# dotnetpower/infomesh

Hardware: AMD Instinct MI355X
Metric: queries/sec (hybrid BM25+dense search, 1.25M docs) (higher is better)
Workload: dtype bf16; 1 GPU; model=bge-small-en(random-init) encoder + BM25 CSR + cosine top-k, global_batch=128, seq_len=32, parallelism=shard1, mode=hybrid, docs_per_gpu=1250000, total_docs=1250000

## Files before the change

### infomesh_amd/index/gpu_index.py

```python
from __future__ import annotations

import math
import re
from dataclasses import dataclass

import numpy as np
import torch

from ..hashing import hash64
from .doc_attrs import DEAD_BIT, DocFilter, pack_pred, passes, words_i32

BM25_K1 = 1.2
BM25_B = 0.75
BM25_VOCAB = 1 << 17

MAX_SEGMENTS = 16

_WORD_RE = re.compile(r"\w+")


def bm25_term_ids(text: str, vocab: int = BM25_VOCAB) -> np.ndarray:
    from ..utils.plugins import GLOBAL_PLUGINS
    tok = GLOBAL_PLUGINS.get_single("tokenizer")
    if tok is not None:
# ... 26 lines not shown
class PostingSegment:
    offsets: torch.Tensor
    doc_ids: torch.Tensor
    tfdl: torch.Tensor
    doc_base: int
    n_docs: int
    h_offs: np.ndarray

    def hbm_bytes(self) -> int:
        return sum(t.numel() * t.element_size()
                   for t in (self.offsets, self.doc_ids, self.tfdl))


class GpuShard:

    def __init__(self, device: str = "cuda", vocab: int = BM25_VOCAB,
                 emb_dtype: str = "bf16"):
        assert emb_dtype in ("bf16", "fp8")
        self.device = torch.device(device)
        self.vocab = vocab
        self.emb_dtype = emb_dtype
        self.n_docs = 0
        self.segments: list[PostingSegment] = []
        self.df: np.ndarray = np.zeros(vocab, dtype=np.int64)
        self._doc_lens = np.zeros(0, dtype=np.int64)
        self.avgdl = 1.0
        self._emb_buf: torch.Tensor | None = None
        self._gid_buf: torch.Tensor | None = None
        self._attr_buf: torch.Tensor | None = None
        self.n_dead = 0
        self._live_bits = None
        self._topk = None
        self._topk_dense = None
        self._dense_graphs: dict = {}
        self.graph_dense = False
        self._h_idf: np.ndarray | None = None
        self._pend_tokens: list[np.ndarray] = []
        self._pend_emb: list[torch.Tensor] = []
        self._pend_gids: list[int] = []
        self._pend_attrs: list = []

    @property
    def embeddings(self) -> torch.Tensor | None:
        if self._emb_buf is None or self.n_docs == 0:
            return None
        return self._emb_buf[:self.n_docs]

    @property
    def global_ids(self) -> torch.Tensor | None:
        if self._gid_buf is None:
            return None
        return self._gid_buf[:self.n_docs]

    @property
    def attrs(self) -> torch.Tensor | None:
        if self._attr_buf is None:
            return None
        return self._attr_buf[:self.n_docs]

    @property
    def doc_norm(self) -> torch.Tensor:
        dl = self._doc_lens.astype(np.float32)
        return torch.from_numpy(
            BM25_K1 * (1 - BM25_B + BM25_B * dl / self.avgdl))

    def add_document(self, global_id: int, term_ids: np.ndarray,
# ... 210 lines not shown
        d = torch.from_numpy(np.ascontiguousarray(flat_docs)).to(dev)
        key, _ = torch.sort(t * np.int64(max(n_new, 1)) + d)
        del t, d
        uniq, counts = torch.unique_consecutive(key, return_counts=True)
        del key
        terms_u = uniq // max(n_new, 1)
        docs_u = (uniq % max(n_new, 1)).to(torch.int32)
        del uniq
        tf = counts.clamp(max=65535).to(torch.int32)
        dl_dev = torch.from_numpy(
            np.minimum(doc_lens, 65535).astype(np.int64)).to(dev)
        dl = dl_dev[docs_u.long()].to(torch.int32)
        tfdl = (tf | (dl << 16)).contiguous()
        df_dev = torch.bincount(terms_u, minlength=self.vocab)
        offsets_dev = torch.zeros(self.vocab + 1, dtype=torch.int64,
                                  device=dev)
        torch.cumsum(df_dev, 0, out=offsets_dev[1:])
        df_new = df_dev.cpu().numpy().astype(np.int64)
        seg = PostingSegment(
            offsets=offsets_dev, doc_ids=docs_u.contiguous(),
            tfdl=tfdl, doc_base=self.n_docs, n_docs=n_new,
            h_offs=offsets_dev.cpu().numpy())
        return seg, df_new

    def _upload_t(self, t: torch.Tensor, stream) -> torch.Tensor:
        pinned = t.contiguous().pin_memory()
        with torch.cuda.stream(stream):
            return pinned.to(self.device, non_blocking=True)

    def _invalidate_query_caches(self) -> None:
        self._h_idf = None
        self._dense_graphs = {}
        self._dense_bufs = {}
        self._bm25_hists = {}
        self._live_bits = None

    def optimize(self) -> None:
        if len(self.segments) <= 1:
            return
        dev = self.device
        V = self.vocab
        term_parts, doc_parts, tfdl_parts = [], [], []
        arangeV = torch.arange(V, dtype=torch.int64, device=dev)
        for seg in self.segments:
            dfg = seg.offsets.diff()
            term_parts.append(torch.repeat_interleave(arangeV, dfg))
            doc_parts.append(seg.doc_ids.to(torch.int64) + seg.doc_base)
            tfdl_parts.append(seg.tfdl)
        terms = torch.cat(term_parts)
        docs = torch.cat(doc_parts)
        tfdl = torch.cat(tfdl_parts)
        key = terms * self.n_docs + docs
        key, order = torch.sort(key)
        docs_sorted = (key % self.n_docs).to(torch.int32)
        tfdl_sorted = tfdl[order].contiguous()
        offsets = torch.zeros(V + 1, dtype=torch.int64, device=dev)
        torch.cumsum(torch.from_numpy(self.df).to(dev), 0,
                     out=offsets[1:])
        self.segments = [PostingSegment(
            offsets=offsets, doc_ids=docs_sorted, tfdl=tfdl_sorted,
            doc_base=0, n_docs=self.n_docs,
            h_offs=offsets.cpu().numpy())]
        self._invalidate_query_caches()

    def delete(self, global_ids) -> int:
        ids = np.unique(np.asarray(list(global_ids), dtype=np.int64))
# ... 264 lines not shown
        tp = _time.perf_counter()

        if query_emb is not None and self.embeddings is not None:
            dn_vals, dn_idx = self.search_dense(query_emb, k, mark=mark,
                                                _mask=mask)
        else:
            dn_vals = torch.full((B, k), -float("inf"), device=dev)
            dn_idx = torch.full((B, k), -1, device=dev, dtype=torch.int32)

        return ShardHits(bm25_scores=bm_vals,
                         bm25_ids=self.to_global(bm_idx),
                         dense_scores=dn_vals,
                         dense_ids=self.to_global(dn_idx))

    def search_dense(self, query_emb: torch.Tensor, k: int,
                     mark=None, filters=None, _mask=None
                     ) -> tuple[torch.Tensor, torch.Tensor]:
        import time as _time
        from ..ops import kernels as K
        if mark is None:
            def mark(name, t0):
                return t0
        B = query_emb.shape[0]
        N = self.n_docs
        k = min(k, N)
        mask = _mask if _mask is not None else self._mask_for(filters, B)
        tp = _time.perf_counter()
        emb = self.embeddings
        if self.device.type == "cuda" and self.graph_dense and mask is None:
            g = self._dense_graphs.get((B, k))
            if g is None:
                from ..ops.graphs import GraphedCallable

                def _plane(e, _B=B, _k=k, _emb=emb, _tk=K.TopK(self.device)):
                    return _tk(self._dense_gemm(e, _emb, _B, self.n_docs), _k)
                g = self._dense_graphs[(B, k)] = GraphedCallable(_plane)
            vals, idx = g(query_emb.bfloat16())
            out = (vals.clone(), idx.clone())
            mark("shard.dense+topk", tp)
            return out
        d_scores = self._dense_gemm(query_emb, emb, B, N)
        tp = mark("shard.dense", tp)
        if mask is None:
            out = self._get_topk_dense()(d_scores, k)
        else:
            out = self._get_topk_dense()(d_scores, k, mask=mask[0],
                                         row_pred=mask[1])
        mark("shard.densetopk", tp)
        return out

    def _dense_gemm(self, query_emb: torch.Tensor, emb: torch.Tensor,
                    B: int, N: int) -> torch.Tensor:
        from ..ops import kernels as K
        buf = self._get_dense_buf(B)
        if self.emb_dtype == "fp8":
            qa = query_emb
            if qa.dtype != torch.float8_e4m3fn:
                qa = qa.float().to(torch.float8_e4m3fn)
            out2d = buf.reshape(B, N)
            for m0 in range(0, B, 128):
                m1 = min(m0 + 128, B)
                r = K.dense_scores_fp8(qa[m0:m1].contiguous(), emb,
                                       out=out2d[m0:m1])
                assert r is not None, "fp8 dense plane shape ineligible"
            return out2d
        return K.gemm_nt(query_emb.bfloat16().unsqueeze(0), emb,
                         out_f32=True, out=buf).reshape(B, N)

    def _get_dense_buf(self, B: int) -> torch.Tensor:
        N = self.n_docs
        bufs = getattr(self, "_dense_bufs", None)
        if bufs is None:
            bufs = self._dense_bufs = {}
        buf = bufs.get(B)
        if buf is None or buf.shape != (1, B, N):
            buf = bufs[B] = torch.empty(
                1, B, N, device=self.device, dtype=torch.float32)
        return buf

    def to_global(self, idx: torch.Tensor) -> torch.Tensor:
        safe = idx.clamp(min=0).long()
        g = self.global_ids[safe]
        return torch.where(idx >= 0, g, torch.full_like(g, -1))


class CpuShard(GpuShard):

    def __init__(self, vocab: int = BM25_VOCAB, emb_dtype: str = "bf16"):
        super().__init__(device="cpu", vocab=vocab, emb_dtype=emb_dtype)

    def _fail_rows(self, filters, B: int) -> torch.Tensor | None:
        pr = self._pred_rows(filters, B)
        if pr is None:
            return None
        preds, rows = pr
        a = self.attrs.numpy()
        ok = np.stack([passes(a, p) for p in preds.view(np.uint32)])
        return torch.from_numpy(~ok[rows])
# ... 54 lines not shown
```

### infomesh_amd/ops/_ext.py

```python
from __future__ import annotations

import ctypes
from ctypes import c_float, c_int, c_long, c_void_p
from pathlib import Path

from ..errors import GpuExtensionMissing

_LIB: ctypes.CDLL | None = None
_LOAD_ERROR: str | None = None

_SIGNATURES: dict[str, list] = {
    "infomesh_gemm_bf16_nt": [c_void_p, c_void_p, c_void_p, c_void_p,
                              c_int, c_int, c_int, c_int,
                              c_long, c_long, c_long,
                              c_int, c_float, c_int, c_void_p],
    "infomesh_layernorm": [c_void_p, c_void_p, c_void_p, c_void_p,
                           c_void_p, c_void_p, c_long, c_int, c_float,
                           c_void_p],
    "infomesh_rmsnorm": [c_void_p, c_void_p, c_void_p, c_void_p,
                         c_void_p, c_long, c_int, c_float, c_void_p],
    "infomesh_softmax": [c_void_p, c_void_p, c_void_p, c_long, c_int,
                         c_int, c_int, c_float, c_void_p],
    "infomesh_bias_act": [c_void_p, c_void_p, c_long, c_int, c_int, c_void_p],
    "infomesh_silu_mul": [c_void_p, c_void_p, c_void_p, c_long, c_void_p],
# ... 31 lines not shown
                             c_float, c_void_p],
    "infomesh_attn_decode_split": [c_void_p, c_void_p, c_void_p, c_void_p,
                                   c_void_p, c_void_p, c_int, c_int, c_int,
                                   c_int, c_int, c_int, c_float, c_void_p],
    "infomesh_attn_fused": [c_void_p, c_void_p, c_void_p, c_void_p,
                            c_void_p, c_int, c_int, c_int, c_int, c_int,
                            c_int, c_long, c_long, c_long, c_long, c_long,
                            c_long, c_long, c_long, c_long,
                            c_int, c_float, c_void_p],
    "infomesh_kv_append": [c_void_p, c_void_p, c_void_p, c_void_p,
                           c_void_p, c_int, c_int, c_int, c_int, c_void_p],
    "infomesh_dense_scores": [c_void_p, c_void_p, c_void_p,
                              c_int, c_long, c_int, c_float, c_void_p],
    "infomesh_dense_scores_fp8": [c_void_p, c_void_p, c_void_p,
                                  c_int, c_long, c_int, c_float,
                                  c_void_p],
    "infomesh_gemm8_bf16_nt": [c_void_p, c_void_p, c_void_p, c_void_p,
                               c_int, c_int, c_int, c_int,
                               c_long, c_long, c_long,
                               c_int, c_float, c_int, c_void_p],
    "infomesh_gemv_bf16_nt": [c_void_p, c_void_p, c_void_p, c_void_p,
                              c_int, c_int, c_int, c_int,
                              c_long, c_long, c_long,
                              c_int, c_float, c_int, c_void_p],
    "infomesh_qkv_split": [c_void_p, c_void_p, c_void_p, c_void_p,
                           c_void_p, c_void_p, c_void_p,
                           c_int, c_int, c_int, c_int, c_int, c_int,
                           c_void_p],
    "infomesh_merge_heads": [c_void_p, c_void_p, c_int, c_int, c_int,
                             c_int, c_void_p],
    "infomesh_silu_mul_fused": [c_void_p, c_void_p, c_long, c_int,
                                c_void_p],
    "infomesh_gemm_tile": [c_int, c_int, c_int, c_int],
}

_RESTYPES = {"infomesh_topk_workspace_u32": c_long,
             "infomesh_topk_zero_u32": c_long,
             "infomesh_dense_scores": c_int,
             "infomesh_dense_scores_fp8": c_int,
             "infomesh_gemm_tile": c_int}


def _try_load() -> ctypes.CDLL | None:
    global _LOAD_ERROR
    so = Path(__file__).resolve().parent / "libinfomesh_hip.so"
    if not so.exists():
        _LOAD_ERROR = f"{so} not built"
        return None
    try:
        lib = ctypes.CDLL(str(so))
    except OSError as e:
        _LOAD_ERROR = str(e)
        return None
    for name, argtypes in _SIGNATURES.items():
        fn = getattr(lib, name)
        fn.argtypes = argtypes
        fn.restype = _RESTYPES.get(name)
    import os
    if os.environ.get("INFOMESH_SYNC_DEBUG"):
        return _SyncDebugLib(lib)
    return lib


class _SyncDebugLib:

    def __init__(self, real: ctypes.CDLL):
        self._real = real

    def __getattr__(self, name: str):
        fn = getattr(self._real, name)
# ... 37 lines not shown
```

### infomesh_amd/ops/csrc/gemm.hip

```cpp
#include "gemm_common.h"
#include <cstdlib>

namespace {

template <int BM, int BN, int BK, bool OUT_F32>
__global__ __launch_bounds__(256) void gemm_bf16_nt_kernel(
    const bf16* __restrict__ A, const bf16* __restrict__ B,
    void* __restrict__ C, const float* __restrict__ bias,
    int M, int N, int K,
    long strideA, long strideB, long strideC,
    int act, float alpha) {
  __shared__ bf16 smem[2][(BM + BN) * BK];

  const int tiles_n = (N + BN - 1) / BN;
  const int tiles_m = (M + BM - 1) / BM;
  const int tile = xcd_swizzle(blockIdx.x, tiles_m * tiles_n);
  const int tm = tile / tiles_n, tn = tile % tiles_n;
  const int m0 = tm * BM, n0 = tn * BN;
  const int g = blockIdx.y;

  const bf16* Ag = A + (long)g * strideA;
  const bf16* Bg = B + (long)g * strideB;

  const int tid = threadIdx.x;
  const int lane = tid & 63;
  const int wid = tid >> 6;
  constexpr int WM = (BM == 128 || BN == 64) ? 2 : 1;
  constexpr int WN = 4 / WM;
  constexpr int FM = (BM / WM) / 16;
  constexpr int FN = (BN / WN) / 16;
  const int wm = wid / WN, wn = wid % WN;

  constexpr int CHUNKS = ((BM > BN ? BM : BN) * BK * 2) / 1024;
  constexpr int CHUNKS_PER_WAVE = CHUNKS / 4;
  constexpr int ACHUNKS = (BM * BK * 2) / 1024;
  constexpr int BCHUNKS2 = (BN * BK * 2) / 1024;

  const int n_ksteps = K / BK;

  auto stage = [&](int buf, int kstep) {
    const long k0 = (long)kstep * BK;
#pragma unroll
    for (int c = 0; c < CHUNKS_PER_WAVE; ++c) {
      const int chunk = wid * CHUNKS_PER_WAVE + c;
// ... 30 lines not shown
  for (int t = 0; t < n_ksteps; ++t) {
    if (t + 1 < n_ksteps) stage(cur ^ 1, t + 1);
#pragma unroll
    for (int ks = 0; ks < BK / 32; ++ks) {
      bf16x8 a[FM], b[FN];
#pragma unroll
      for (int i = 0; i < FM; ++i) {
        const int row = wm * (BM / WM) + i * 16 + fr;
        const int off = (row * BK + ks * 32 + fk) * 2;
        a[i] = *reinterpret_cast<const bf16x8*>(
            (const char*)&smem[cur][0]
            + ((BK == 64) ? swz(off) : off));
      }
#pragma unroll
      for (int j = 0; j < FN; ++j) {
        const int row = wn * (BN / WN) + j * 16 + fr;
        const int off = (row * BK + ks * 32 + fk) * 2;
        b[j] = *reinterpret_cast<const bf16x8*>(
            (const char*)&smem[cur][BM * BK]
            + ((BK == 64) ? swz(off) : off));
      }
#pragma unroll
      for (int i = 0; i < FM; ++i)
#pragma unroll
        for (int j = 0; j < FN; ++j)
          acc[i][j] = __builtin_amdgcn_mfma_f32_16x16x32_bf16(
              a[i], b[j], acc[i][j], 0, 0, 0);
    }
    __syncthreads();
    cur ^= 1;
  }

  const int m_base = m0 + wm * (BM / WM), n_base = n0 + wn * (BN / WN);
  if (OUT_F32 && n0 + BN <= N && m0 + BM <= M) {
    float* stage_f32 = reinterpret_cast<float*>(&smem[0][0])
        + wid * (BM / WM) * (BN / WN);
    __syncthreads();
    store_frags_staged_f32(acc, stage_f32, reinterpret_cast<float*>(C),
                           (long)g * strideC, bias, m_base, n_base, N,
                           act, alpha, lane);
    return;
  }
  store_frags_guarded<OUT_F32>(acc, C, (long)g * strideC, bias,
                               m_base, n_base, M, N, N, act, alpha, lane);
}

template <bool OUT_F32>
__global__ __launch_bounds__(256) void gemm_pipe64_kernel(
    const bf16* __restrict__ A, const bf16* __restrict__ B,
    void* __restrict__ C, const float* __restrict__ bias,
    int M, int N, int K,
    long strideA, long strideB, long strideC,
    int act, float alpha) {
  constexpr int BM = 64, BN = 64, BK = 64;
  __shared__ bf16 smem[3][(BM + BN) * BK];

  const int tiles_n = (N + BN - 1) / BN;
  const int tiles_m = (M + BM - 1) / BM;
  const int tile = xcd_swizzle(blockIdx.x, tiles_m * tiles_n);
  const int m0 = (tile / tiles_n) * BM, n0 = (tile % tiles_n) * BN;
  const int g = blockIdx.y;
  const bf16* Ag = A + (long)g * strideA;
  const bf16* Bg = B + (long)g * strideB;

  const int lane = threadIdx.x & 63;
  const int wid = threadIdx.x >> 6;
  const int wm = wid >> 1, wn = wid & 1;
  constexpr int FN = BN / 2 / 16;
  const int n_ksteps = K / BK;

  constexpr int CPW = (BM + BN) * BK * 2 / 1024 / 4;
  auto stage = [&](int buf, int t) {
    const int ks = t < n_ksteps ? t : n_ksteps - 1;
    const long k0 = (long)ks * BK;
#pragma unroll
    for (int c = 0; c < CPW; ++c) {
      const int chunk = wid * CPW + c;
// ... 87 lines not shown
  bool pipe;
};

GemmTile pick_tile(int M, int N, int K, int batch, int force) {
  int bm = (M <= 64) ? 64 : 128, bn = 128;
  const long blocks128 =
      (long)((M + 127) / 128) * ((N + 127) / 128) * batch;
  if (bm == 128 && blocks128 < 512 && K <= 2048) bm = bn = 64;
  if (force == 64 && M > 64) bm = bn = 64;
  else if (force == 128) bm = bn = 128;
  const int bk = (K % 64 == 0) ? 64 : 32;
  return {bm, bn, bk, bm == 64 && bn == 64 && bk == 64};
}

GemmKernel tile_kernel(GemmTile t, bool out_f32) {
  if (t.pipe)
    return out_f32 ? gemm_pipe64_kernel<true> : gemm_pipe64_kernel<false>;
  if (t.bn == 64) return generic_kernel<64, 64, 32>(out_f32);
  if (t.bm == 64)
    return t.bk == 64 ? generic_kernel<64, 128, 64>(out_f32)
                      : generic_kernel<64, 128, 32>(out_f32);
  return t.bk == 64 ? generic_kernel<128, 128, 64>(out_f32)
                    : generic_kernel<128, 128, 32>(out_f32);
}

int tile_override() {
  static const int ov = [] {
    const char* e = getenv("INFOMESH_GEMM_TILE");
    return e ? atoi(e) : -1;
  }();
  return ov;
}

}

extern "C" int infomesh_gemm_tile(int M, int N, int K, int batch) {
  const GemmTile t = pick_tile(M, N, K, batch, tile_override());
  return t.bm | t.bn << 8 | t.bk << 16 | (int)t.pipe << 24;
}

extern "C" void infomesh_gemm_bf16_nt(
    const void* A, const void* B, void* C, const void* bias,
    int M, int N, int K, int batch,
    long strideA, long strideB, long strideC,
    int act, float alpha, int out_f32, void* stream) {
  const GemmTile t = pick_tile(M, N, K, batch, tile_override());
  const int tiles = ((M + t.bm - 1) / t.bm) * ((N + t.bn - 1) / t.bn);
  hipLaunchKernelGGL(tile_kernel(t, out_f32), dim3(tiles, batch), dim3(256),
                     0, reinterpret_cast<hipStream_t>(stream),
                     (const bf16*)A, (const bf16*)B, C, (const float*)bias,
                     M, N, K, strideA, strideB, strideC, act, alpha);
}
```

### infomesh_amd/ops/csrc/gemm_common.h

```cpp
#pragma once
#include "common.h"

DEVINL int swz(int byte_off) {
  return byte_off ^ ((((byte_off >> 7) ^ (byte_off >> 10)) & 7) << 4);
}

template <int CPOL>
DEVINL void glds16(const bf16* gsrc, void* lds_base) {
  __builtin_amdgcn_global_load_lds(
      (const __attribute__((address_space(1))) unsigned int*)gsrc,
      (__attribute__((address_space(3))) unsigned int*)lds_base,
      16, 0, CPOL);
}


template <bool OUT_F32, int FM, int FN>
DEVINL void store_frags_guarded(const f32x4 (&acc)[FM][FN], void* C,
                                long c_off, const float* bias,
                                int m_base, int n_base, int M, int N,
                                int ldc, int act, float alpha, int lane) {
  const int crow_base = (lane >> 4) * 4;
  const int ccol = lane & 15;
#pragma unroll
  for (int i = 0; i < FM; ++i) {
#pragma unroll
    for (int j = 0; j < FN; ++j) {
      const int n = n_base + j * 16 + ccol;
      if (n >= N) continue;
      const float bv = bias ? bias[n] : 0.0f;
#pragma unroll
      for (int r = 0; r < 4; ++r) {
        const int m = m_base + i * 16 + crow_base + r;
        if (m >= M) continue;
        float v = apply_act(alpha * acc[i][j][r] + bv, act);
        if (OUT_F32)
          reinterpret_cast<float*>(C)[c_off + (long)m * ldc + n] = v;
        else
          reinterpret_cast<bf16*>(C)[c_off + (long)m * ldc + n] = f2bf(v);
      }
    }
  }
}

template <int FM, int FN>
DEVINL void store_frags_staged_f32(const f32x4 (&acc)[FM][FN],
                                   float* stage_f32, float* C, long c_off,
                                   const float* bias, int m_base,
                                   int n_base, int N, int act,
                                   float alpha, int lane) {
  constexpr int SEGN = FN * 16;
  const int crow_base = (lane >> 4) * 4;
  const int ccol = lane & 15;
#pragma unroll
  for (int i = 0; i < FM; ++i)
#pragma unroll
    for (int j = 0; j < FN; ++j)
#pragma unroll
      for (int r = 0; r < 4; ++r) {
        const int lm = i * 16 + crow_base + r;
        const int ln = j * 16 + ccol;
        const float bv = bias ? bias[n_base + ln] : 0.0f;
        stage_f32[lm * SEGN + ln] =
            apply_act(alpha * acc[i][j][r] + bv, act);
      }
  asm volatile("s_waitcnt lgkmcnt(0)" ::: "memory");
  __builtin_amdgcn_wave_barrier();
  constexpr int LPR = SEGN * 4 / 16;
  constexpr int ROWS_PER_IT = 64 / LPR;
  const int srow = lane / LPR, scol4 = (lane % LPR) * 4;
#pragma unroll
  for (int base = 0; base < FM * 16; base += ROWS_PER_IT) {
    const int lm = base + srow;
    const int m = m_base + lm;
    const int n = n_base + scol4;
    f32x4 v = *reinterpret_cast<const f32x4*>(
        &stage_f32[lm * SEGN + scol4]);
    __builtin_nontemporal_store(
        v, reinterpret_cast<f32x4*>(C + c_off + (long)m * N + n));
  }
}
```

### infomesh_amd/ops/csrc/topk.hip

```cpp
#include "common.h"

#define TOPK_CAP 8192

#define HI_RES 4096

namespace {

struct MaskRef {
  const unsigned* bits;
  const int* row_pred;
  long W;
};
DEVINL const unsigned* mask_row(const MaskRef& m, int b) {
  return m.bits + (long)m.row_pred[b] * m.W;
}
DEVINL unsigned mask_nibble(const unsigned* __restrict__ mrow, long i) {
  return (mrow[i >> 3] >> ((unsigned)(i & 7) * 4)) & 15u;
}
DEVINL void keep_loaded(float4& v) {
  asm volatile("" : "+v"(v.x), "+v"(v.y), "+v"(v.z), "+v"(v.w));
}
DEVINL bool mask_bit(const unsigned* __restrict__ mrow, long col) {
  return (mrow[col >> 5] >> (unsigned)(col & 31)) & 1u;
}
// ... 240 lines not shown
    for (int j = k >> 1; j > 0; j >>= 1) {
      for (int i = threadIdx.x; i < n2; i += blockDim.x) {
        const int ixj = i ^ j;
        if (ixj > i) {
          const bool up = ((i & k) == 0);
          const unsigned long long a = d[i], c = d[ixj];
          if ((a > c) == up) { d[i] = c; d[ixj] = a; }
        }
      }
      __syncthreads();
    }
  }
  for (int i = threadIdx.x; i < K; i += blockDim.x) {
    if (i < n) {
      const unsigned long long v = d[i];
      out_vals[(long)b * K + i] = ordered_to_float(~(unsigned)(v >> 32));
      out_idx[(long)b * K + i] = (int)(v & 0xffffffffu);
    } else {
      out_vals[(long)b * K + i] = -INFINITY;
      out_idx[(long)b * K + i] = -1;
    }
  }
}

struct TopkLayout {
  long hist1, hist2, bin1, chi1, thresh, shift, cnt, cnt_eq, cand, total;
  explicit TopkLayout(long B)
      : hist1(0), hist2(hist1 + B * 256), bin1(hist2 + B * 256),
        chi1(bin1 + B), thresh(chi1 + B), shift(thresh + B),
        cnt(shift + B), cnt_eq(cnt + B),
        cand((cnt_eq + B + 1) & ~1L),
        total(cand + B * TOPK_CAP * 2) {}
};

}

extern "C" long infomesh_topk_workspace_u32(int B) {
  return TopkLayout(B).total;
}

extern "C" long infomesh_topk_zero_u32(int B) { return TopkLayout(B).cand; }

template <bool MASKED, typename... M>
static void topk_launch(const void* scores, void* workspace, void* out_vals,
                        void* out_idx, int B, long N, int K,
                        const void* ext_hist1, hipStream_t s, M... mask) {
  static_assert(sizeof...(M) == (MASKED ? 1 : 0), "one MaskRef iff MASKED");
  unsigned* ws = reinterpret_cast<unsigned*>(workspace);
  const TopkLayout L(B);
  auto* cand = reinterpret_cast<unsigned long long*>(ws + L.cand);

  int chunks = (int)min((N + 256 * 64 - 1) / (256 * 64), (long)1024);
  if (chunks < 1) chunks = 1;
  dim3 g1(chunks, B), blk(256);
  const unsigned* h1 = (const unsigned*)ext_hist1;
  if (!h1) {
    h1 = ws + L.hist1;
    hipLaunchKernelGGL((hist1_kernel<MASKED, M...>), g1, blk, 0, s,
                       (const float*)scores, ws + L.hist1, N, mask...);
  }
  hipLaunchKernelGGL(select1_kernel, dim3(B), dim3(64), 0, s,
                     h1, ws + L.bin1, ws + L.chi1, K);
  hipLaunchKernelGGL((hist2_kernel<MASKED, M...>), g1, blk, 0, s,
                     (const float*)scores, ws + L.bin1, ws + L.hist2, N,
                     mask...);
  hipLaunchKernelGGL((select2_kernel<MASKED, M...>), dim3(B),
                     dim3(SELECT2_THREADS), 0, s, (const float*)scores,
                     ws + L.hist2, ws + L.bin1, ws + L.chi1, ws + L.thresh,
                     ws + L.shift, N, K, mask...);
  hipLaunchKernelGGL((compact_kernel<MASKED, M...>), g1, blk, 0, s,
                     (const float*)scores, ws + L.thresh, ws + L.shift, cand,
                     ws + L.cnt, ws + L.cnt_eq, N, mask...);
  hipLaunchKernelGGL(sort_emit_kernel, dim3(B), blk, 0, s,
                     cand, ws + L.cnt, ws + L.cnt_eq, (float*)out_vals,
                     (int*)out_idx, K);
}

extern "C" void infomesh_topk(const void* scores, void* workspace,
                              void* out_vals, void* out_idx,
                              int B, long N, int K,
                              const void* ext_hist1, void* stream) {
  topk_launch<false>(scores, workspace, out_vals, out_idx, B, N, K,
                     ext_hist1, reinterpret_cast<hipStream_t>(stream));
}

extern "C" void infomesh_topk_masked(const void* scores, void* workspace,
                                     void* out_vals, void* out_idx,
                                     int B, long N, int K,
                                     const void* bits, const void* row_pred,
                                     long W, void* stream) {
  topk_launch<true>(scores, workspace, out_vals, out_idx, B, N, K, nullptr,
                    reinterpret_cast<hipStream_t>(stream),
                    MaskRef{(const unsigned*)bits, (const int*)row_pred, W});
}
```

### infomesh_amd/ops/kernels.py

```python
from __future__ import annotations

import torch

from . import _ext

ACT = {"none": 0, "gelu": 1, "silu": 2, "relu": 3, "tanh": 4}


def _ptr(t: torch.Tensor | None) -> int | None:
    return None if t is None else t.data_ptr()


def _check(t: torch.Tensor, dtype: torch.dtype, name: str) -> None:
    assert t.is_cuda, f"{name} must be on GPU"
    assert t.dtype == dtype, f"{name} must be {dtype}, got {t.dtype}"
    assert t.is_contiguous(), f"{name} must be contiguous"


def gemm_route(M: int, N: int, K: int, G: int) -> str:
    if M <= 16:
        return "gemv"
    if (M >= 4096 and N >= 512 and K % 64 == 0
            and ((M + 255) // 256) * ((N + 255) // 256) * max(G, 1) >= 224):
        return "gemm8"
# ... 14 lines not shown
            bias: torch.Tensor | None = None,
            act: str = "none", alpha: float = 1.0,
            out_f32: bool = False,
            out: torch.Tensor | None = None) -> torch.Tensor:
    sq_a = a.dim() == 2
    if sq_a:
        a = a.unsqueeze(0)
    if b.dim() == 2:
        b = b.unsqueeze(0).expand(a.shape[0], *b.shape)
    G, M, K = a.shape
    Gb, N, Kb = b.shape
    assert K == Kb and Gb == G, f"shape mismatch {a.shape} x {b.shape}"
    assert K % 32 == 0, f"K={K} must be a multiple of 32"
    _check(a, torch.bfloat16, "A")
    assert b.dtype == torch.bfloat16
    strideB = 0 if (G > 1 and b.stride(0) == 0) else N * K
    if strideB != 0:
        assert b.is_contiguous()
    else:
        assert b[0].is_contiguous()
    if bias is not None:
        _check(bias, torch.float32, "bias")
        assert bias.numel() == N
    dtype = torch.float32 if out_f32 else torch.bfloat16
    if out is None:
        out = torch.empty((G, M, N), device=a.device, dtype=dtype)
    else:
        assert out.shape == (G, M, N) and out.dtype == dtype and out.is_contiguous()
    fn = getattr(_ext.lib(), _GEMM_ENTRY[gemm_route(M, N, K, G)])
    fn(a.data_ptr(), b.data_ptr(), out.data_ptr(), _ptr(bias),
       M, N, K, G, M * K, strideB, M * N,
       ACT[act], alpha, int(out_f32), _ext.stream_ptr())
    return out.squeeze(0) if sq_a else out


def dense_scores(a: torch.Tensor, b: torch.Tensor, alpha: float = 1.0,
                 out: torch.Tensor | None = None) -> torch.Tensor | None:
    M, K = a.shape
    N = b.shape[0]
    _check(a, torch.bfloat16, "A")
    _check(b, torch.bfloat16, "B")
    if out is None:
        out = torch.empty(M, N, device=a.device, dtype=torch.float32)
    rc = _ext.lib().infomesh_dense_scores(
        a.data_ptr(), b.data_ptr(), out.data_ptr(), M, N, K, alpha,
        _ext.stream_ptr())
    return out if rc == 0 else None


def dense_scores_fp8(a: torch.Tensor, b: torch.Tensor,
                     alpha: float = 1.0,
                     out: torch.Tensor | None = None
                     ) -> torch.Tensor | None:
    M, K = a.shape
    N = b.shape[0]
    assert a.dtype == torch.float8_e4m3fn and a.is_cuda and a.is_contiguous()
    assert b.dtype == torch.float8_e4m3fn and b.is_contiguous()
    if out is None:
        out = torch.empty(M, N, device=a.device, dtype=torch.float32)
    rc = _ext.lib().infomesh_dense_scores_fp8(
        a.data_ptr(), b.data_ptr(), out.data_ptr(), M, N, K, alpha,
        _ext.stream_ptr())
    return out if rc == 0 else None


def layernorm(x: torch.Tensor, gamma: torch.Tensor, beta: torch.Tensor,
# ... 141 lines not shown
        assert 1 <= k <= 1024
        assert (mask is None) == (row_pred is None), \
            "mask and row_pred go together"
        if mask is not None:
            assert ext_hist1 is None, "ext_hist1 cannot be masked"
            _check(mask, torch.int32, "mask")
            _check(row_pred, torch.int32, "row_pred")
            assert mask.dim() == 2 and mask.shape[1] * 32 >= N
            assert row_pred.numel() == B
        if ext_hist1 is not None:
            assert ext_hist1.dtype == torch.int32 \
                and ext_hist1.numel() >= B * 256
        lib = _ext.lib()
        nu32 = lib.infomesh_topk_workspace_u32(B)
        if self._ws is None or self._ws.numel() < nu32:
            self._ws = torch.empty(nu32, device=scores.device,
                                   dtype=torch.int32)
        self._ws[:lib.infomesh_topk_zero_u32(B)].zero_()
        vals = torch.empty((B, k), device=scores.device, dtype=torch.float32)
        idx = torch.empty((B, k), device=scores.device, dtype=torch.int32)
        if mask is not None:
            lib.infomesh_topk_masked(
                scores.data_ptr(), self._ws.data_ptr(), vals.data_ptr(),
                idx.data_ptr(), B, N, k, mask.data_ptr(),
                row_pred.data_ptr(), mask.shape[1], _ext.stream_ptr())
            return vals, idx
        lib.infomesh_topk(scores.data_ptr(), self._ws.data_ptr(),
                          vals.data_ptr(), idx.data_ptr(), B, N, k,
                          0 if ext_hist1 is None else ext_hist1.data_ptr(),
                          _ext.stream_ptr())
        return vals, idx


def topk(scores: torch.Tensor, k: int) -> tuple[torch.Tensor, torch.Tensor]:
    return TopK(scores.device)(scores, k)


def filter_bitmask(attrs: torch.Tensor, preds: torch.Tensor) -> torch.Tensor:
    _check(attrs, torch.int32, "attrs")
    _check(preds, torch.int32, "preds")
    assert attrs.dim() == 2 and attrs.shape[1] == 4
    assert preds.dim() == 2 and preds.shape[1] == 4 and preds.shape[0] >= 1
    N, P = attrs.shape[0], preds.shape[0]
    assert P <= 65535
    W = (N + 63) // 64 * 2
    bits = torch.empty((P, W), device=attrs.device, dtype=torch.int32)
    _ext.lib().infomesh_filter_bitmask(
        attrs.data_ptr(), preds.data_ptr(), bits.data_ptr(), N, P,
        _ext.stream_ptr())
    return bits


def bm25_block(doc_ids: torch.Tensor, tfdl: torch.Tensor,
               qt_off: torch.Tensor, qt_ut: torch.Tensor,
               qt_idf: torch.Tensor, u_begin: torch.Tensor,
               u_end: torch.Tensor, bounds: torch.Tensor,
               scores: torch.Tensor, doc_base: int, nseg: int,
               bd: int, avgdl: float, k1: float = 1.2,
               b: float = 0.75,
               hist1: torch.Tensor | None = None) -> torch.Tensor:
    B, N = scores.shape
    U = u_begin.numel()
    nblocks = (nseg + bd - 1) // bd
    _check(scores, torch.float32, "scores")
    assert nblocks <= 65535 and qt_off.numel() == B + 1
    assert doc_ids.dtype == torch.int32 and tfdl.dtype == torch.int32
# ... 152 lines not shown
```

### infomesh_amd/ops/reference.py

```python
from __future__ import annotations

import torch


def gemm_nt(a: torch.Tensor, b: torch.Tensor,
            bias: torch.Tensor | None = None, act: str = "none",
            alpha: float = 1.0) -> torch.Tensor:
    out = alpha * torch.matmul(a.float(), b.float().transpose(-1, -2))
    if bias is not None:
        out = out + bias.float()
    return apply_act(out, act)


def apply_act(x: torch.Tensor, act: str) -> torch.Tensor:
    if act == "gelu":
        return torch.nn.functional.gelu(x, approximate="tanh")
    if act == "silu":
        return torch.nn.functional.silu(x)
    if act == "relu":
        return torch.relu(x)
    if act == "tanh":
        return torch.tanh(x)
    return x

# ... 113 lines not shown
                out.add((m, n))
    return out


def filter_bitmask(attrs: torch.Tensor, preds: torch.Tensor) -> torch.Tensor:
    import numpy as np
    from ..index.doc_attrs import passes
    a = attrs.cpu().numpy()
    N = a.shape[0]
    W = (N + 63) // 64 * 2
    rows = []
    for pred in preds.cpu().numpy().view(np.uint32):
        ok = np.zeros(W * 32, dtype=bool)
        ok[:N] = passes(a, pred)
        rows.append(np.packbits(ok, bitorder="little").view(np.uint32))
    return torch.from_numpy(np.stack(rows).view(np.int32).reshape(-1, W))


def masked_topk(scores: torch.Tensor, k: int, bits: torch.Tensor,
                row_pred: torch.Tensor) -> tuple[torch.Tensor, torch.Tensor]:
    import numpy as np
    B, N = scores.shape
    words = bits.cpu().numpy().view(np.uint32)
    ok = np.unpackbits(words.view(np.uint8), axis=1,
                       bitorder="little")[:, :N].astype(bool)
    ok = torch.from_numpy(ok[row_pred.cpu().numpy().astype(np.int64)])
    s = scores.detach().float().cpu().masked_fill(~ok, float("-inf"))
    vals, idx = torch.topk(s, k, dim=1)
    idx = torch.where(torch.isinf(vals) & (vals < 0),
                      torch.full_like(idx, -1), idx)
    return vals, idx


def attn_decode(q: torch.Tensor, k_cache: torch.Tensor,
                v_cache: torch.Tensor, lens: torch.Tensor,
                scale: float) -> torch.Tensor:
    B, H, D = q.shape
    _, Hkv, Smax, _ = k_cache.shape
    group = H // Hkv
    out = torch.zeros_like(q, dtype=torch.float32)
    for b in range(B):
        L = int(lens[b])
        for h in range(H):
            kv = h // group
            k = k_cache[b, kv, :L].float()
            v = v_cache[b, kv, :L].float()
            p = torch.softmax(q[b, h].float() @ k.T * scale, dim=-1)
            out[b, h] = p @ v
    return out
```

Measured before the change: 40570 queries/s.

## Fuse per-block score maxima into dense GEMM and prune top-k to candidate blocks

The dense GEMM epilogue now also writes the maximum score of each W-wide column block per query row, using DPP cross-lane max reductions. Top-k then runs first over these block maxima to pick K candidate blocks, gathers only those blocks' scores, runs a second small top-k, and maps indices back to document ids. This avoids a full radix top-k pass over all 1.25M scores per query. The cost is extra epilogue work in the GEMM, several extra small kernel launches, and more workspace.

```diff
diff --git a/infomesh_amd/index/gpu_index.py b/infomesh_amd/index/gpu_index.py
--- a/infomesh_amd/index/gpu_index.py
+++ b/infomesh_amd/index/gpu_index.py
@@ -82,6 +82,8 @@
         self._live_bits = None
         self._topk = None
         self._topk_dense = None
+        self._topk_pruned = None
+        self._dense_bmax: dict = {}
         self._dense_graphs: dict = {}
         self.graph_dense = False
         self._h_idf: np.ndarray | None = None
@@ -358,6 +360,7 @@
         self._h_idf = None
         self._dense_graphs = {}
         self._dense_bufs = {}
+        self._dense_bmax = {}
         self._bm25_hists = {}
         self._live_bits = None
 
@@ -688,25 +691,38 @@
             if g is None:
                 from ..ops.graphs import GraphedCallable
 
-                def _plane(e, _B=B, _k=k, _emb=emb, _tk=K.TopK(self.device)):
-                    return _tk(self._dense_gemm(e, _emb, _B, self.n_docs), _k)
+                def _plane(e, _B=B, _k=k, _emb=emb,
+                           _tk=(K.TopK(self.device),
+                                K.TopKPruned(self.device))):
+                    return self._dense_select(
+                        self._dense_gemm(e, _emb, _B, self.n_docs), _k, *_tk)
                 g = self._dense_graphs[(B, k)] = GraphedCallable(_plane)
             vals, idx = g(query_emb.bfloat16())
             out = (vals.clone(), idx.clone())
             mark("shard.dense+topk", tp)
             return out
-        d_scores = self._dense_gemm(query_emb, emb, B, N)
+        d_scores = self._dense_gemm(query_emb, emb, B, N,
+                                    with_bmax=mask is None)
         tp = mark("shard.dense", tp)
         if mask is None:
-            out = self._get_topk_dense()(d_scores, k)
+            if self._topk_pruned is None:
+                self._topk_pruned = K.TopKPruned(self.device)
+            out = self._dense_select(d_scores, k, self._get_topk_dense(),
+                                     self._topk_pruned)
         else:
             out = self._get_topk_dense()(d_scores, k, mask=mask[0],
                                          row_pred=mask[1])
         mark("shard.densetopk", tp)
         return out
 
+    @staticmethod
+    def _dense_select(d_scores, k: int, topk, topk_pruned):
+        if isinstance(d_scores, tuple):
+            return topk_pruned(*d_scores, k)
+        return topk(d_scores, k)
+
     def _dense_gemm(self, query_emb: torch.Tensor, emb: torch.Tensor,
-                    B: int, N: int) -> torch.Tensor:
+                    B: int, N: int, with_bmax: bool = True):
         from ..ops import kernels as K
         buf = self._get_dense_buf(B)
         if self.emb_dtype == "fp8":
@@ -720,6 +736,15 @@
                                        out=out2d[m0:m1])
                 assert r is not None, "fp8 dense plane shape ineligible"
             return out2d
+        W = K.gemm_bmax_width(B, N, emb.shape[1]) if with_bmax else 0
+        if W:
+            bmax = self._dense_bmax.get(B)
+            if bmax is None or bmax.shape != (B, (N + W - 1) // W):
+                bmax = self._dense_bmax[B] = torch.empty(
+                    B, (N + W - 1) // W, device=self.device,
+                    dtype=torch.float32)
+            return K.gemm_nt_bmax(query_emb.bfloat16().contiguous(), emb,
+                                  out=buf.reshape(B, N), bmax=bmax)
         return K.gemm_nt(query_emb.bfloat16().unsqueeze(0), emb,
                          out_f32=True, out=buf).reshape(B, N)
 
diff --git a/infomesh_amd/ops/_ext.py b/infomesh_amd/ops/_ext.py
--- a/infomesh_amd/ops/_ext.py
+++ b/infomesh_amd/ops/_ext.py
@@ -87,10 +87,23 @@
     "infomesh_silu_mul_fused": [c_void_p, c_void_p, c_long, c_int,
                                 c_void_p],
     "infomesh_gemm_tile": [c_int, c_int, c_int, c_int],
+    "infomesh_gemm_bmax_width": [c_int, c_int, c_int, c_int],
+    "infomesh_gemm_bf16_nt_bmax": [c_void_p, c_void_p, c_void_p, c_void_p,
+                                   c_void_p, c_int, c_int, c_int, c_int,
+                                   c_long, c_long, c_long,
+                                   c_int, c_float, c_void_p],
+    "infomesh_topk_pruned": [c_void_p, c_void_p, c_int, c_void_p, c_void_p,
+                             c_void_p, c_int, c_long, c_int, c_void_p],
+    "infomesh_topk_pruned_workspace_u32": [c_int, c_long, c_int, c_int],
+    "infomesh_topk_pruned_zero_u32": [c_int],
 }
 
 _RESTYPES = {"infomesh_topk_workspace_u32": c_long,
              "infomesh_topk_zero_u32": c_long,
+             "infomesh_topk_pruned_workspace_u32": c_long,
+             "infomesh_topk_pruned_zero_u32": c_long,
+             "infomesh_gemm_bmax_width": c_int,
+             "infomesh_gemm_bf16_nt_bmax": c_int,
              "infomesh_dense_scores": c_int,
              "infomesh_dense_scores_fp8": c_int,
              "infomesh_gemm_tile": c_int}
diff --git a/infomesh_amd/ops/csrc/gemm.hip b/infomesh_amd/ops/csrc/gemm.hip
--- a/infomesh_amd/ops/csrc/gemm.hip
+++ b/infomesh_amd/ops/csrc/gemm.hip
@@ -3,13 +3,19 @@
 
 namespace {
 
-template <int BM, int BN, int BK, bool OUT_F32>
+__host__ DEVINL long bmax_blocks(int N, int W) { return ((long)N + W - 1) / W; }
+DEVINL float* bmax_of(float* p) { return p; }
+
+template <int BM, int BN, int BK, bool OUT_F32, bool BMAX = false,
+          typename... BmaxPtr>
 __global__ __launch_bounds__(256) void gemm_bf16_nt_kernel(
     const bf16* __restrict__ A, const bf16* __restrict__ B,
     void* __restrict__ C, const float* __restrict__ bias,
     int M, int N, int K,
     long strideA, long strideB, long strideC,
-    int act, float alpha) {
+    int act, float alpha, BmaxPtr... bmax) {
+  static_assert(sizeof...(BmaxPtr) == (BMAX ? 1 : 0) && (OUT_F32 || !BMAX),
+                "one float* iff BMAX, and BMAX is f32 only");
   __shared__ bf16 smem[2][(BM + BN) * BK];
 
   const int tiles_n = (N + BN - 1) / BN;
@@ -106,17 +112,32 @@
   }
 
   const int m_base = m0 + wm * (BM / WM), n_base = n0 + wn * (BN / WN);
-  if (OUT_F32 && n0 + BN <= N && m0 + BM <= M) {
+  constexpr bool STAGE_FITS = BM * BN * 4 <= (int)sizeof(smem);
+  if (OUT_F32 && STAGE_FITS && n0 + BN <= N && m0 + BM <= M) {
     float* stage_f32 = reinterpret_cast<float*>(&smem[0][0])
         + wid * (BM / WM) * (BN / WN);
     __syncthreads();
-    store_frags_staged_f32(acc, stage_f32, reinterpret_cast<float*>(C),
-                           (long)g * strideC, bias, m_base, n_base, N,
-                           act, alpha, lane);
+    if constexpr (BMAX)
+      store_frags_staged_f32<FM, FN, true>(
+          acc, stage_f32, reinterpret_cast<float*>(C), (long)g * strideC,
+          bias, m_base, n_base, N, act, alpha, lane,
+          bmax_of(bmax...) + (long)g * M * bmax_blocks(N, BN / WN),
+          bmax_blocks(N, BN / WN));
+    else
+      store_frags_staged_f32(acc, stage_f32, reinterpret_cast<float*>(C),
+                             (long)g * strideC, bias, m_base, n_base, N,
+                             act, alpha, lane);
     return;
   }
-  store_frags_guarded<OUT_F32>(acc, C, (long)g * strideC, bias,
-                               m_base, n_base, M, N, N, act, alpha, lane);
+  if constexpr (BMAX)
+    store_frags_guarded_bmax(
+        acc, reinterpret_cast<float*>(C), (long)g * strideC, bias, m_base,
+        n_base, M, N, act, alpha, lane,
+        bmax_of(bmax...) + (long)g * M * bmax_blocks(N, BN / WN),
+        bmax_blocks(N, BN / WN));
+  else
+    store_frags_guarded<OUT_F32>(acc, C, (long)g * strideC, bias,
+                                 m_base, n_base, M, N, N, act, alpha, lane);
 }
 
 template <bool OUT_F32>
@@ -270,6 +291,24 @@
   return ov;
 }
 
+GemmTile bmax_tile(int M, int K, int force) {
+  if (force == 64 && M > 64) return {0, 0, 0, false};
+  return {(M <= 64 && force != 128) ? 64 : 128, 128,
+          (K % 64 == 0) ? 64 : 32, false};
+}
+int bmax_width(GemmTile t) { return t.bm == 0 ? 0 : t.bm == 128 ? 64 : 32; }
+
+template <int BM, int BK>
+void launch_bmax(dim3 grid, hipStream_t s, const void* A, const void* B,
+                 void* C, const void* bias, void* bmax, int M, int N, int K,
+                 long strideA, long strideB, long strideC, int act,
+                 float alpha) {
+  hipLaunchKernelGGL((gemm_bf16_nt_kernel<BM, 128, BK, true, true, float*>),
+                     grid, dim3(256), 0, s, (const bf16*)A, (const bf16*)B,
+                     C, (const float*)bias, M, N, K, strideA, strideB,
+                     strideC, act, alpha, (float*)bmax);
+}
+
 }
 
 extern "C" int infomesh_gemm_tile(int M, int N, int K, int batch) {
@@ -289,3 +328,23 @@
                      (const bf16*)A, (const bf16*)B, C, (const float*)bias,
                      M, N, K, strideA, strideB, strideC, act, alpha);
 }
+
+extern "C" int infomesh_gemm_bmax_width(int M, int N, int K, int batch) {
+  return bmax_width(bmax_tile(M, K, tile_override()));
+}
+
+extern "C" int infomesh_gemm_bf16_nt_bmax(
+    const void* A, const void* B, void* C, const void* bias, void* bmax,
+    int M, int N, int K, int batch,
+    long strideA, long strideB, long strideC,
+    int act, float alpha, void* stream) {
+  const GemmTile t = bmax_tile(M, K, tile_override());
+  if (bmax_width(t) == 0) return 1;
+  const dim3 grid(((M + t.bm - 1) / t.bm) * ((N + t.bn - 1) / t.bn), batch);
+  auto* launch = t.bm == 128
+      ? (t.bk == 64 ? launch_bmax<128, 64> : launch_bmax<128, 32>)
+      : (t.bk == 64 ? launch_bmax<64, 64> : launch_bmax<64, 32>);
+  launch(grid, reinterpret_cast<hipStream_t>(stream), A, B, C, bias, bmax,
+         M, N, K, strideA, strideB, strideC, act, alpha);
+  return 0;
+}
diff --git a/infomesh_amd/ops/csrc/gemm_common.h b/infomesh_amd/ops/csrc/gemm_common.h
--- a/infomesh_amd/ops/csrc/gemm_common.h
+++ b/infomesh_amd/ops/csrc/gemm_common.h
@@ -42,12 +42,28 @@
   }
 }
 
-template <int FM, int FN>
+template <int CTRL>
+DEVINL uint32_t max_dpp(uint32_t v) {
+  return max(v, (uint32_t)__builtin_amdgcn_update_dpp((int)v, (int)v, CTRL,
+                                                      0xf, 0xf, false));
+}
+template <int G>
+DEVINL uint32_t group_max_u32(uint32_t o) {
+  static_assert(G == 8 || G == 16, "a half or a whole DPP row");
+  o = max_dpp<0xB1>(o);
+  o = max_dpp<0x4E>(o);
+  o = max_dpp<0x141>(o);
+  if (G == 16) o = max_dpp<0x140>(o);
+  return o;
+}
+
+template <int FM, int FN, bool BMAX = false>
 DEVINL void store_frags_staged_f32(const f32x4 (&acc)[FM][FN],
                                    float* stage_f32, float* C, long c_off,
                                    const float* bias, int m_base,
                                    int n_base, int N, int act,
-                                   float alpha, int lane) {
+                                   float alpha, int lane,
+                                   float* bmax = nullptr, long NB = 0) {
   constexpr int SEGN = FN * 16;
   const int crow_base = (lane >> 4) * 4;
   const int ccol = lane & 15;
@@ -67,7 +83,10 @@
   __builtin_amdgcn_wave_barrier();
   constexpr int LPR = SEGN * 4 / 16;
   constexpr int ROWS_PER_IT = 64 / LPR;
+  static_assert(!BMAX || FM * 16 == LPR * ROWS_PER_IT,
+                "BMAX: 64 rows per wave, one maximum per lane");
   const int srow = lane / LPR, scol4 = (lane % LPR) * 4;
+  uint32_t mine = 0;
 #pragma unroll
   for (int base = 0; base < FM * 16; base += ROWS_PER_IT) {
     const int lm = base + srow;
@@ -77,5 +96,55 @@
         &stage_f32[lm * SEGN + scol4]);
     __builtin_nontemporal_store(
         v, reinterpret_cast<f32x4*>(C + c_off + (long)m * N + n));
+    if constexpr (BMAX) {
+      const uint32_t o = group_max_u32<LPR>(
+          max(max(float_to_ordered(v[0]), float_to_ordered(v[1])),
+              max(float_to_ordered(v[2]), float_to_ordered(v[3]))));
+      if (lane % LPR == base / ROWS_PER_IT) mine = o;
+    }
+  }
+  if constexpr (BMAX) {
+    const int m = m_base + (lane % LPR) * ROWS_PER_IT + srow;
+    bmax[(long)m * NB + n_base / SEGN] = ordered_to_float(mine);
   }
 }
+
+template <int FM, int FN>
+DEVINL void store_frags_guarded_bmax(const f32x4 (&acc)[FM][FN], float* C,
+                                     long c_off, const float* bias,
+                                     int m_base, int n_base, int M, int N,
+                                     int act, float alpha, int lane,
+                                     float* bmax, long NB) {
+  static_assert(FM == 4, "64 rows per wave, one maximum per lane");
+  constexpr int SEGN = FN * 16;
+  const int crow_base = (lane >> 4) * 4;
+  const int ccol = lane & 15;
+  uint32_t mine = 0;
+#pragma unroll
+  for (int i = 0; i < FM; ++i) {
+    uint32_t o[4] = {0u, 0u, 0u, 0u};
+#pragma unroll
+    for (int j = 0; j < FN; ++j) {
+      const int n = n_base + j * 16 + ccol;
+      const bool valid = n < N;
+      const float bv = (valid && bias) ? bias[n] : 0.0f;
+#pragma unroll
+      for (int r = 0; r < 4; ++r) {
+        const int m = m_base + i * 16 + crow_base + r;
+        const float v = apply_act(alpha * acc[i][j][r] + bv, act);
+        if (valid) {
+          o[r] = max(o[r], float_to_ordered(v));
+          if (m < M) C[c_off + (long)m * N + n] = v;
+        }
+      }
+    }
+#pragma unroll
+    for (int r = 0; r < 4; ++r) {
+      const uint32_t g = group_max_u32<16>(o[r]);
+      if (ccol == i * 4 + r) mine = g;
+    }
+  }
+  const int m = m_base + (ccol >> 2) * 16 + crow_base + (ccol & 3);
+  if (m < M && n_base < N)
+    bmax[(long)m * NB + n_base / SEGN] = ordered_to_float(mine);
+}
diff --git a/infomesh_amd/ops/csrc/topk.hip b/infomesh_amd/ops/csrc/topk.hip
--- a/infomesh_amd/ops/csrc/topk.hip
+++ b/infomesh_amd/ops/csrc/topk.hip
@@ -296,6 +296,74 @@
         cand((cnt_eq + B + 1) & ~1L),
         total(cand + B * TOPK_CAP * 2) {}
 };
+unsigned long long* cand_of(unsigned* ws, long B) {
+  return reinterpret_cast<unsigned long long*>(ws + TopkLayout(B).cand);
+}
+
+#define PRUNE_THREADS 1024
+#define PRUNE_PAD 0xffffffffu
+__global__ __launch_bounds__(PRUNE_THREADS) void gather_blocks_kernel(
+    const float* __restrict__ scores, const int* __restrict__ ids,
+    int* __restrict__ blk, float* __restrict__ gath, long N, long NB,
+    int W, int K1) {
+  __shared__ int d[1024];
+  const int b = blockIdx.x;
+  int n2 = 64;
+  while (n2 < K1) n2 <<= 1;
+  for (int i = threadIdx.x; i < n2; i += blockDim.x)
+    d[i] = i < K1 ? ids[(long)b * K1 + i] : 0x7fffffff;
+  __syncthreads();
+  for (int k = 2; k <= n2; k <<= 1) {
+    for (int j = k >> 1; j > 0; j >>= 1) {
+      for (int i = threadIdx.x; i < n2; i += blockDim.x) {
+        const int ixj = i ^ j;
+        if (ixj > i) {
+          const bool up = ((i & k) == 0);
+          const int a = d[i], c = d[ixj];
+          if ((a > c) == up) { d[i] = c; d[ixj] = a; }
+        }
+      }
+      __syncthreads();
+    }
+  }
+  for (int i = threadIdx.x; i < K1; i += blockDim.x)
+    blk[(long)b * K1 + i] = d[i];
+  const float* row = scores + (long)b * N;
+  float* grow = gath + (long)b * K1 * W;
+  for (int e = threadIdx.x; e < K1 * W; e += blockDim.x) {
+    const long id = d[e / W];
+    const long col = id * W + e % W;
+    grow[e] = (id >= 0 && id < NB && col < N) ? row[col]
+                                              : __uint_as_float(PRUNE_PAD);
+  }
+}
+
+__global__ __launch_bounds__(256) void remap_blocks_kernel(
+    const int* __restrict__ blk, float* __restrict__ out_vals,
+    int* __restrict__ out_idx, long N, int W, int K1, int K) {
+  const int b = blockIdx.x;
+  for (int i = threadIdx.x; i < K; i += blockDim.x) {
+    const int p = out_idx[(long)b * K + i];
+    if (p < 0) continue;
+    const long col = (long)blk[(long)b * K1 + p / W] * W + p % W;
+    if (col < N) {
+      out_idx[(long)b * K + i] = (int)col;
+    } else {
+      out_vals[(long)b * K + i] = -INFINITY;
+      out_idx[(long)b * K + i] = -1;
+    }
+  }
+}
+
+struct PrunedLayout {
+  long K1, zero2, cand, vals1, idx1, blk, gath, total;
+  PrunedLayout(long B, long NB, long K, long W)
+      : K1(K < NB ? K : NB), zero2(TopkLayout(B).cand), cand(2 * zero2),
+        vals1(cand + B * TOPK_CAP * 2), idx1(vals1 + B * K1),
+        blk(idx1 + B * K1),
+        gath((blk + B * K1 + 3) & ~3L),
+        total(gath + B * K1 * W) {}
+};
 
 }
 
@@ -306,13 +374,12 @@
 extern "C" long infomesh_topk_zero_u32(int B) { return TopkLayout(B).cand; }
 
 template <bool MASKED, typename... M>
-static void topk_launch(const void* scores, void* workspace, void* out_vals,
+static void topk_launch(const void* scores, unsigned* ws,
+                        unsigned long long* cand, void* out_vals,
                         void* out_idx, int B, long N, int K,
                         const void* ext_hist1, hipStream_t s, M... mask) {
   static_assert(sizeof...(M) == (MASKED ? 1 : 0), "one MaskRef iff MASKED");
-  unsigned* ws = reinterpret_cast<unsigned*>(workspace);
   const TopkLayout L(B);
-  auto* cand = reinterpret_cast<unsigned long long*>(ws + L.cand);
 
   int chunks = (int)min((N + 256 * 64 - 1) / (256 * 64), (long)1024);
   if (chunks < 1) chunks = 1;
@@ -344,7 +411,8 @@
                               void* out_vals, void* out_idx,
                               int B, long N, int K,
                               const void* ext_hist1, void* stream) {
-  topk_launch<false>(scores, workspace, out_vals, out_idx, B, N, K,
+  unsigned* ws = reinterpret_cast<unsigned*>(workspace);
+  topk_launch<false>(scores, ws, cand_of(ws, B), out_vals, out_idx, B, N, K,
                      ext_hist1, reinterpret_cast<hipStream_t>(stream));
 }
 
@@ -353,7 +421,39 @@
                                      int B, long N, int K,
                                      const void* bits, const void* row_pred,
                                      long W, void* stream) {
-  topk_launch<true>(scores, workspace, out_vals, out_idx, B, N, K, nullptr,
-                    reinterpret_cast<hipStream_t>(stream),
+  unsigned* ws = reinterpret_cast<unsigned*>(workspace);
+  topk_launch<true>(scores, ws, cand_of(ws, B), out_vals, out_idx, B, N, K,
+                    nullptr, reinterpret_cast<hipStream_t>(stream),
                     MaskRef{(const unsigned*)bits, (const int*)row_pred, W});
 }
+
+extern "C" long infomesh_topk_pruned_workspace_u32(int B, long N, int K,
+                                                   int W) {
+  return PrunedLayout(B, (N + W - 1) / W, K, W).total;
+}
+extern "C" long infomesh_topk_pruned_zero_u32(int B) {
+  return 2 * TopkLayout(B).cand;
+}
+
+extern "C" void infomesh_topk_pruned(const void* scores, const void* bmax,
+                                     int W, void* workspace, void* out_vals,
+                                     void* out_idx, int B, long N, int K,
+                                     void* stream) {
+  hipStream_t s = reinterpret_cast<hipStream_t>(stream);
+  unsigned* ws = reinterpret_cast<unsigned*>(workspace);
+  const long NB = (N + W - 1) / W;
+  const PrunedLayout L(B, NB, K, W);
+  const int K1 = (int)L.K1;
+  auto* cand = reinterpret_cast<unsigned long long*>(ws + L.cand);
+  int* idx1 = reinterpret_cast<int*>(ws + L.idx1);
+  int* blk = reinterpret_cast<int*>(ws + L.blk);
+  float* gath = reinterpret_cast<float*>(ws + L.gath);
+  topk_launch<false>(bmax, ws, cand, ws + L.vals1, idx1, B, NB, K1, nullptr,
+                     s);
+  hipLaunchKernelGGL(gather_blocks_kernel, dim3(B), dim3(PRUNE_THREADS), 0,
+                     s, (const float*)scores, idx1, blk, gath, N, NB, W, K1);
+  topk_launch<false>(gath, ws + L.zero2, cand, out_vals, out_idx, B,
+                     (long)K1 * W, K, nullptr, s);
+  hipLaunchKernelGGL(remap_blocks_kernel, dim3(B), dim3(256), 0, s, blk,
+                     (float*)out_vals, (int*)out_idx, N, W, K1, K);
+}
diff --git a/infomesh_amd/ops/kernels.py b/infomesh_amd/ops/kernels.py
--- a/infomesh_amd/ops/kernels.py
+++ b/infomesh_amd/ops/kernels.py
@@ -70,6 +70,40 @@
        M, N, K, G, M * K, strideB, M * N,
        ACT[act], alpha, int(out_f32), _ext.stream_ptr())
     return out.squeeze(0) if sq_a else out
+
+
+def gemm_bmax_width(M: int, N: int, K: int, G: int = 1) -> int:
+    if gemm_route(M, N, K, G) != "gemm":
+        return 0
+    return _ext.lib().infomesh_gemm_bmax_width(M, N, K, G)
+
+
+def gemm_nt_bmax(a: torch.Tensor, b: torch.Tensor, alpha: float = 1.0,
+                 out: torch.Tensor | None = None,
+                 bmax: torch.Tensor | None = None
+                 ) -> tuple[torch.Tensor, torch.Tensor, int] | None:
+    M, K = a.shape
+    N, Kb = b.shape
+    assert K == Kb and K % 32 == 0, f"shape mismatch {a.shape} x {b.shape}"
+    _check(a, torch.bfloat16, "A")
+    _check(b, torch.bfloat16, "B")
+    W = gemm_bmax_width(M, N, K)
+    if W == 0:
+        return None
+    NB = (N + W - 1) // W
+    if out is None:
+        out = torch.empty((M, N), device=a.device, dtype=torch.float32)
+    if bmax is None:
+        bmax = torch.empty((M, NB), device=a.device, dtype=torch.float32)
+    for t, shape, name in ((out, (M, N), "out"), (bmax, (M, NB), "bmax")):
+        _check(t, torch.float32, name)
+        assert t.shape == shape, f"{name} must be {shape}, got {t.shape}"
+    rc = _ext.lib().infomesh_gemm_bf16_nt_bmax(
+        a.data_ptr(), b.data_ptr(), out.data_ptr(), None, bmax.data_ptr(),
+        M, N, K, 1, M * K, N * K, M * N, ACT["none"], alpha,
+        _ext.stream_ptr())
+    assert rc == 0, "tile changed between gemm_bmax_width and the launch"
+    return out, bmax, W
 
 
 def dense_scores(a: torch.Tensor, b: torch.Tensor, alpha: float = 1.0,
@@ -277,6 +311,35 @@
         return vals, idx
 
 
+class TopKPruned:
+
+    def __init__(self, device: torch.device | str = "cuda"):
+        self.device = torch.device(device)
+        self._ws: torch.Tensor | None = None
+
+    def __call__(self, scores: torch.Tensor, bmax: torch.Tensor, W: int,
+                 k: int) -> tuple[torch.Tensor, torch.Tensor]:
+        assert scores.dim() == 2
+        _check(scores, torch.float32, "scores")
+        _check(bmax, torch.float32, "bmax")
+        B, N = scores.shape
+        assert 1 <= k <= 1024 and W > 0
+        assert bmax.shape == (B, (N + W - 1) // W), \
+            f"bmax must be [B, ceil(N/W)], got {tuple(bmax.shape)}"
+        lib = _ext.lib()
+        nu32 = lib.infomesh_topk_pruned_workspace_u32(B, N, k, W)
+        if self._ws is None or self._ws.numel() < nu32:
+            self._ws = torch.empty(nu32, device=scores.device,
+                                   dtype=torch.int32)
+        self._ws[:lib.infomesh_topk_pruned_zero_u32(B)].zero_()
+        vals = torch.empty((B, k), device=scores.device, dtype=torch.float32)
+        idx = torch.empty((B, k), device=scores.device, dtype=torch.int32)
+        lib.infomesh_topk_pruned(
+            scores.data_ptr(), bmax.data_ptr(), W, self._ws.data_ptr(),
+            vals.data_ptr(), idx.data_ptr(), B, N, k, _ext.stream_ptr())
+        return vals, idx
+
+
 def topk(scores: torch.Tensor, k: int) -> tuple[torch.Tensor, torch.Tensor]:
     return TopK(scores.device)(scores, k)
 
diff --git a/infomesh_amd/ops/reference.py b/infomesh_amd/ops/reference.py
--- a/infomesh_amd/ops/reference.py
+++ b/infomesh_amd/ops/reference.py
@@ -169,6 +169,48 @@
     return vals, idx
 
 
+def ordered_key(x: torch.Tensor) -> torch.Tensor:
+    bits = x.detach().float().cpu().contiguous().view(torch.int32) \
+        .to(torch.int64) & 0xFFFFFFFF
+    return torch.where(bits >= 0x80000000, bits ^ 0xFFFFFFFF,
+                       bits | 0x80000000)
+
+
+def block_max(scores: torch.Tensor, W: int) -> torch.Tensor:
+    s = scores.detach().float().cpu()
+    B, N = s.shape
+    NB = (N + W - 1) // W
+    key = torch.full((B, NB * W), -1, dtype=torch.int64)
+    key[:, :N] = ordered_key(s)
+    pos = key.view(B, NB, W).argmax(dim=2)
+    cols = (pos + torch.arange(NB) * W).clamp(max=N - 1)
+    return s.gather(1, cols)
+
+
+def topk_pruned(scores: torch.Tensor, bmax: torch.Tensor, W: int,
+                k: int) -> tuple[torch.Tensor, torch.Tensor]:
+    s = scores.detach().float().cpu()
+    B, N = s.shape
+    NB = (N + W - 1) // W
+    assert bmax.shape == (B, NB)
+    k1 = min(k, NB)
+    ids = torch.topk(ordered_key(bmax), k1, dim=1).indices.sort(dim=1).values
+    cols = (ids[:, :, None] * W + torch.arange(W)).reshape(B, k1 * W)
+    real = cols < N
+    cand = s.gather(1, cols.clamp(max=N - 1))
+    key = torch.where(real, ordered_key(cand), torch.full_like(cols, -1))
+    key = torch.where(key == 0x7FFFFFFF, key + 1, key)
+    order = torch.sort(key, dim=1, descending=True, stable=True).indices
+    kk = min(k, k1 * W)
+    order = order[:, :kk]
+    vals = torch.full((B, k), float("-inf"))
+    idx = torch.full((B, k), -1, dtype=torch.int64)
+    ok = real.gather(1, order)
+    vals[:, :kk] = torch.where(ok, cand.gather(1, order), vals[:, :kk])
+    idx[:, :kk] = torch.where(ok, cols.gather(1, order), idx[:, :kk])
+    return vals, idx
+
+
 def attn_decode(q: torch.Tensor, k_cache: torch.Tensor,
                 v_cache: torch.Tensor, lens: torch.Tensor,
                 scale: float) -> torch.Tensor:
```

Result: faster. 43550 queries/s (median of 6 runs) (+7.3%).
